# mpetri/ans-large-alphabet

Measured on AMD Instinct MI355X. Metric: encode+decode Mints/s (uint32), bit-exact vs CPU reference per block, higher is better.
Workload: dtype u32 symbols; ANS state carried as an exact f64 (integers below 2^53) in the encoder, u64 in the decoder; 1 GPU; ANSfold-1 on 268435456 uint32 per GPU, zipf20s1.2, blocks of 16384 ints, restart every 1024; codec=ANSfold-1, ints_per_gpu=268435456, distribution=zipf20s1.2, block_ints=16384, ckpt_interval=1024, seed=1234, multi_gpu=single GPU

## Files before the change

### ans_large_alphabet_amd/csrc/ansx.hip

```cpp
#include "../../include/ansx.h"

#include <hip/hip_runtime.h>
#include <dlfcn.h>
#include <rccl/rccl.h>

#include <algorithm>
#include <array>
#include <cmath>
#include <cstdio>
#include <cstdlib>
#include <cstring>
#include <deque>
#include <functional>
#include <map>
#include <set>
#include <string>
#include <vector>

#include "ansx_kernels.h"
#include "ansx_rfold.h"
#include "ansx_model.h"
#include "ansx_fastmodel.h"
#include "ansx_gen.h"
#include "ansx_pa.h"
// ... 67 lines not shown
    std::vector<hipEvent_t> pipe_ev;
    struct {
        bool table16_fixup = false;
        bool encode_gtab16 = false;
        bool parse_generic = false;
        bool parse_win = false;
        bool parse_fast = false;
        bool decode_table = false;
        bool no_stream_lds = false;
        int decode_mode = 0;
        u32 parse_stage_words = 0;
        bool model_fused = false;
        bool model_sync = false;
        bool use_pc = false;
        u32 pc_b_pairs = 2;
        u32 test_sp_bits = 0;
        bool fin_one_wave = false;
        bool no_big_geo = false;
        bool no_pc_auto = false;
        bool encode_mode2 = false;
        bool force_pc = false;
        bool no_pc = false;
        int decode_small_ring = 0;
        int decode_pair = 0;
        u32 pair_lds_limit = 0;
        u32 wide_at = 16;
        bool wide_restart = false;
        u32 ns_hint = 0;
        u32 t_hint = 0;
        bool no_fast_model = false;
        double near_band = ANSX_NEAR_BAND;
        bool near_flip = false;
        u32 cand_chains = 0;
        double fast_guard = ANSX_FAST_GUARD;
        int model_pipeline = 0;
        u32 batch_pass_blocks = 0;
    } dbg;
};

namespace {

#define HIPCHK(ctx, call)                                                                        \
    do {                                                                                         \
        hipError_t _e = (call);                                                                  \
        if (_e != hipSuccess) {                                                                  \
            (ctx)->last_hip = (int)_e;                                                           \
// ... 1171 lines not shown
        const u64 key = geo_key(P.g);
        const size_t stream_bound = block_bound(P.g.kind, P.g.f, P.g.block_ints, P.g.pa != 0) + 16;
        const bool must = P.g.kind == ANSX_INT || stream_bound >= ((size_t)1 << ANSX_CK_CURSOR_BITS) || c->dbg.wide_restart;
        const bool hinted = !must && c->wide_hint.count(key) != 0;
        set_restart_format(&P, must || hinted);
        int rc = encode_dev_once(c, P, d_in, d_out, cap, out_bytes, s);
        if (rc == ANSX_OK && hinted && c->last.max_log2_frame <= c->dbg.wide_at) {
            c->wide_hint.erase(key);
            set_restart_format(&P, false);
            const u32 path0 = c->last.path;
            rc = encode_dev_once(c, P, d_in, d_out, cap, out_bytes, s);
            c->last.path |= (path0 & 16u) | 64u;
        }
        if (rc != ANSX_RETRY_WIDE) return rc;
        c->wide_hint.insert(key);
        set_restart_format(&P, true);
        const int rc2 = encode_dev_once(c, P, d_in, d_out, cap, out_bytes, s);
        c->last.path |= 32u;
        return rc2;
    }
    return encode_dev_once(c, P, d_in, d_out, cap, out_bytes, s);
}

template <bool RF>
int launch_decode(ansx_ctx* c, const ansx_geo& g, u32 NSP, const u8* cont, const u64* boff,
    const u64* ck_state, const u32* ck_off, u64 payload_off, u32* d_out, u32 maxM, u32 max_ns,
    u32 max_block_bytes, u64 cont_bytes, u32* gflags, hipStream_t s, const uint4* pa_info, const u32* hints, u32 max_ep,
    bool parsed = false)
{
    const u32 T = fold_T(g.f);
    int rc;
    if ((rc = ensure(c, c->dec_cum, (size_t)g.nblocks * (NSP + 8) * 4))) return rc;
    if ((rc = ensure(c, c->dec_info, (size_t)g.nblocks * 16))) return rc;
    const size_t pf_e = std::max<size_t>(20480, rup(((size_t)max_ns + 2) * 128, 16));
    const size_t pf_lds = pf_e + (size_t)ANSX_PF_SW * 64 * 4 + 21 * 64 * 4;
    u32 stage_words = ANSX_PF_SW;
    if (c->dbg.parse_stage_words >= 2 && c->dbg.parse_stage_words <= ANSX_PF_SW)
        stage_words = c->dbg.parse_stage_words & ~1u;
    if (parsed) {
    } else if (c->dbg.parse_generic) {
        LAUNCH(c, "k_parse_prelude", (k_parse_prelude<RF>), (g.nblocks + 63) / 64, 64, 0, s, cont, g, NSP,
            boff, payload_off, max_ns, maxM, (u32*)c->dec_cum.p, (uint4*)c->dec_info.p, gflags, pa_info);
    } else if (hints != nullptr && !c->dbg.parse_win && !c->dbg.parse_fast) {
        const u32 par_waves = (g.nblocks + 7) / 8;
        const u32 pw_max = max_ns <= 1024 ? 3u : 4u;
        const u32 pw = std::min<u32>(pw_max, std::max<u32>(1u, (par_waves + c->num_cus - 1) / c->num_cus));
        const u32 par_grid = (par_waves + pw - 1) / pw;
        const size_t lds = (size_t)pw * (32 + 48) * 64 * 4;
        HIPCHK(c, hipFuncSetAttribute((const void*)k_parse_prelude_par<RF, 32>,
                      hipFuncAttributeMaxDynamicSharedMemorySize, (int)lds));
        LAUNCH(c, "k_parse_prelude", (k_parse_prelude_par<RF, 32>), par_grid, 64 * pw, lds, s, cont, g, NSP, boff,
            payload_off, max_ns, maxM, hints, (u32*)c->dec_cum.p, (uint4*)c->dec_info.p, gflags, pa_info);
    } else if (c->dbg.parse_fast && (u64)maxM + max_ns + 3 <= 65535u && pf_lds <= 150 * 1024) {
        HIPCHK(c, hipFuncSetAttribute((const void*)k_parse_prelude_fast<RF>,
                      hipFuncAttributeMaxDynamicSharedMemorySize, (int)pf_lds));
        LAUNCH(c, "k_parse_prelude", (k_parse_prelude_fast<RF>), (g.nblocks + 63) / 64, 64, pf_lds, s, cont, g,
            NSP, boff, payload_off, max_ns, maxM, (u32*)c->dec_cum.p, (uint4*)c->dec_info.p, gflags, stage_words, pa_info);
    } else if (max_ns <= 1024) {
        const size_t lds = (size_t)(128 + 72) * 64 * 4;
        HIPCHK(c, hipFuncSetAttribute((const void*)k_parse_prelude_win<RF, 128>,
                      hipFuncAttributeMaxDynamicSharedMemorySize, (int)lds));
        LAUNCH(c, "k_parse_prelude", (k_parse_prelude_win<RF, 128>), (g.nblocks + 63) / 64, 64, lds, s, cont, g,
            NSP, boff, payload_off, max_ns, maxM, (u32*)c->dec_cum.p, (uint4*)c->dec_info.p, gflags, pa_info);
    } else {
        const size_t lds = (size_t)(256 + 72) * 64 * 4;
        HIPCHK(c, hipFuncSetAttribute((const void*)k_parse_prelude_win<RF, 256>,
                      hipFuncAttributeMaxDynamicSharedMemorySize, (int)lds));
        LAUNCH(c, "k_parse_prelude", (k_parse_prelude_win<RF, 256>), (g.nblocks + 63) / 64, 64, lds, s, cont, g,
            NSP, boff, payload_off, max_ns, maxM, (u32*)c->dec_cum.p, (uint4*)c->dec_info.p, gflags, pa_info);
    }
    const u32 nseg = geo_nseg(g.block_ints, g.ckpt);
    u32 threads = (u32)rup((size_t)nseg * 4, 64);
    if (threads > 256) threads = 256;
    const size_t mfb = RF ? (size_t)T * 4 : 0;
    const size_t want_stream = rup((size_t)max_block_bytes + 32, 16);
    const size_t LDS_LIMIT = 150 * 1024;
    const size_t rs_tables = rup((size_t)(maxM >= 32 ? maxM / 32 : 1) * 8, 16) + 2 * rup((size_t)max_ep * 4, 16) + ANSX_DEC_SCRATCH;
    if (maxM <= 65536u && rs_tables <= LDS_LIMIT && !c->dbg.decode_table) {
        const size_t ring_lds = (size_t)(threads / 4) * ANSX_RING_STRIDE + 16;
        const bool staged_fits = rs_tables + want_stream <= 52 * 1024;
        const bool ring_ok = g.ckpt != 0 && g.block_ints % g.ckpt == 0 && g.ckpt % 4 == 0
            && rs_tables + ring_lds <= 60 * 1024;
        const bool ring_pays = !staged_fits || rs_tables >= 12 * 1024
            || 10 * (rs_tables + want_stream) > 16 * (rs_tables + ring_lds);
        const int force = c->dbg.decode_mode;
        const bool use_ring = ring_ok && (force ? force == 1 : ring_pays);
        if (use_ring) {
            const size_t lds2 = rup((size_t)(maxM >= 32 ? maxM / 32 : 1) * 16, 16) + 4 * rup((size_t)max_ep * 4, 16) + ANSX_DEC_SCRATCH + 2 * ring_lds;
            const int pair = c->dbg.decode_pair;
            if (pair != 1 && g.nblocks >= 2 && (pair == 2 ? lds2 <= 150 * 1024 : lds2 <= c->dbg.pair_lds_limit)) {
                if (lds2 > 48 * 1024)
                    HIPCHK(c, hipFuncSetAttribute((const void*)k_decode_rank2<RF>,
                                  hipFuncAttributeMaxDynamicSharedMemorySize, (int)lds2));
                LAUNCH(c, "k_decode", (k_decode_rank2<RF>), (g.nblocks + 1) / 2, threads, lds2, s, cont, g, NSP, boff,
                    ck_state, ck_off, payload_off, d_out, maxM, max_ep, (u64)cont_bytes, (const u32*)c->dec_cum.p,
                    (const uint4*)c->dec_info.p, gflags);
                return ANSX_OK;
            }
            const int small = c->dbg.decode_small_ring;
            const bool lean = g.n != 0 && (double)(cont_bytes - payload_off) / (double)g.n <= 2.0 && g.ckpt % 16 == 0;
            if (small != 1 && (small == 2 || lean)) {
                const size_t ldss = rs_tables + (size_t)(threads / 4) * ANSX_SRING_STRIDE + 16;
                if (ldss > 48 * 1024)
                    HIPCHK(c, hipFuncSetAttribute((const void*)k_decode_rank<RF, 2>, hipFuncAttributeMaxDynamicSharedMemorySize, (int)ldss));
                LAUNCH(c, "k_decode", (k_decode_rank<RF, 2>), g.nblocks, threads, ldss, s, cont, g, NSP, boff,
                    ck_state, ck_off, payload_off, d_out, maxM, max_ep, (u64)cont_bytes, (const u32*)c->dec_cum.p,
                    (const uint4*)c->dec_info.p, gflags);
                return ANSX_OK;
            }
            const size_t lds = rs_tables + ring_lds;
            if (lds > 48 * 1024)
                HIPCHK(c, hipFuncSetAttribute((const void*)k_decode_rank<RF, 1>,
                              hipFuncAttributeMaxDynamicSharedMemorySize, (int)lds));
            LAUNCH(c, "k_decode", (k_decode_rank<RF, 1>), g.nblocks, threads, lds, s, cont, g, NSP, boff,
                ck_state, ck_off, payload_off, d_out, maxM, max_ep, (u64)cont_bytes, (const u32*)c->dec_cum.p,
                (const uint4*)c->dec_info.p, gflags);
            return ANSX_OK;
        }
        size_t lds = rs_tables;
        u32 stream_cap = 0;
        if (staged_fits && !c->dbg.no_stream_lds) {
            lds += want_stream;
            stream_cap = (u32)want_stream;
        }
        if (lds > 48 * 1024)
            HIPCHK(c, hipFuncSetAttribute((const void*)k_decode_rank<RF, 0>,
                          hipFuncAttributeMaxDynamicSharedMemorySize, (int)lds));
        LAUNCH(c, "k_decode", (k_decode_rank<RF, 0>), g.nblocks, threads, lds, s, cont, g, NSP, boff, ck_state,
            ck_off, payload_off, d_out, maxM, max_ep, (u64)stream_cap, (const u32*)c->dec_cum.p,
            (const uint4*)c->dec_info.p, gflags);
        return ANSX_OK;
    }
    const size_t cb = rup(((size_t)max_ns + 2) * 4, 16);
    const size_t s2sb = rup((size_t)maxM * 2, 16);
    const size_t tables = cb + s2sb + mfb;
    if (tables <= LDS_LIMIT) {
        size_t lds = tables;
        u32 stream_cap = 0;
        if (tables + want_stream <= 52 * 1024) {
            lds += want_stream;
            stream_cap = (u32)want_stream;
        }
        if (lds > 48 * 1024)
            HIPCHK(c, hipFuncSetAttribute((const void*)k_decode<true, RF>,
                          hipFuncAttributeMaxDynamicSharedMemorySize, (int)lds));
        LAUNCH(c, "k_decode_table", (k_decode<true, RF>), g.nblocks, threads, lds, s, cont, g, NSP, boff,
            ck_state, ck_off, payload_off, d_out, maxM, max_ns, stream_cap, (u16*)nullptr,
            (u32*)c->dec_cum.p, (const uint4*)c->dec_info.p, gflags);
    } else {
        if ((rc = ensure(c, c->dec_s2s, (size_t)g.nblocks * maxM * 2))) return rc;
        size_t lds = mfb;
        u32 stream_cap = 0;
        if (mfb + want_stream <= 52 * 1024) {
// ... 1124 lines not shown
    if (hipGetDeviceCount(&ndev) != hipSuccess || ndev == 0) return ANSX_ERR_NO_DEVICE;
    if (device < 0) {
        if (hipGetDevice(&device) != hipSuccess) return ANSX_ERR_NO_DEVICE;
    }
    if (device >= ndev) return ANSX_ERR_ARG;
    if (hipSetDevice(device) != hipSuccess) return ANSX_ERR_NO_DEVICE;
    hipDeviceProp_t prop;
    if (hipGetDeviceProperties(&prop, device) != hipSuccess) return ANSX_ERR_NO_DEVICE;
    if (strncmp(prop.gcnArchName, "gfx950", 6) != 0) return ANSX_ERR_NO_DEVICE;
    ansx_ctx* c = new ansx_ctx();
    c->device = device;
    c->num_cus = prop.multiProcessorCount > 0 ? (u32)prop.multiProcessorCount : 256u;
    if (hipStreamCreateWithFlags(&c->stream, hipStreamDefault) != hipSuccess) {
        delete c;
        return ANSX_ERR_HIP;
    }
    if (hipHostMalloc((void**)&c->h_pin, 4096, hipHostMallocDefault) != hipSuccess) {
        (void)hipStreamDestroy(c->stream);
        delete c;
        return ANSX_ERR_HIP;
    }
    static const char* const names[] = { "ANSX_TEST_TABLE16_FIXUP", "ANSX_ENCODE_GTAB16", "ANSX_PARSE_GENERIC", "ANSX_PARSE_WIN", "ANSX_PARSE_FAST",
        "ANSX_DECODE_TABLE", "ANSX_NO_STREAM_LDS", "ANSX_DECODE_MODE", "ANSX_PARSE_STAGE_WORDS", "ANSX_MODEL_FUSED", "ANSX_MODEL_SYNC", "ANSX_NS_HINT", "ANSX_T_HINT", "ANSX_NO_FAST_MODEL", "ANSX_FAST_GUARD", "ANSX_CAND_CHAINS", "ANSX_NEAR_BAND", "ANSX_TEST_NEAR_FLIP", "ANSX_WIDE_RESTART", "ANSX_TEST_WIDE_AT",
        "ANSX_BATCH_PASS_BLOCKS", "ANSX_MODEL_PIPELINE" };
    for (const char* nm : names)
        if (const char* v = getenv(nm)) (void)ansx_debug_set(c, nm, v);
    *out = c;
    return ANSX_OK;
}

int ansx_last_encode_stats(const ansx_ctx* c, ansx_encode_stats* out)
{
    if (!c || !out) return ANSX_ERR_ARG;
    *out = c->last;
#ifdef ANSX_STAMPS
    {
        static unsigned long long h[16 * 256 + 16];
        if (hipMemcpyFromSymbol(h, HIP_SYMBOL(g_stamps), sizeof(h)) == hipSuccess) {
            double acc[16] = {};
            int nn = 0;
#ifdef ANSX_STAMPS_RF
            const int last = 8;
#else
            const int last = 10;
#endif
            for (int w = 0; w < 256; w++) {
                if (!h[w * 16] || !h[w * 16 + last]) continue;
// ... 40 lines not shown
    else if (!strcmp(name, "ANSX_NO_STREAM_LDS")) c->dbg.no_stream_lds = on;
    else if (!strcmp(name, "ANSX_MODEL_FUSED")) c->dbg.model_fused = on;
    else if (!strcmp(name, "ANSX_MODEL_SYNC")) c->dbg.model_sync = on;
    else if (!strcmp(name, "ANSX_DECODE_MODE"))
        c->dbg.decode_mode = !value ? 0 : !strcmp(value, "ring") ? 1 : !strcmp(value, "staged") ? 2 : 0;
    else if (!strcmp(name, "ANSX_PARSE_STAGE_WORDS")) c->dbg.parse_stage_words = value ? (u32)strtoul(value, nullptr, 10) : 0u;
    else if (!strcmp(name, "ANSX_NS_HINT")) c->dbg.ns_hint = value ? (u32)strtoul(value, nullptr, 10) : 0u;
    else if (!strcmp(name, "ANSX_T_HINT")) c->dbg.t_hint = value ? (u32)strtoul(value, nullptr, 10) : 0u;
    else if (!strcmp(name, "ANSX_NO_FAST_MODEL")) c->dbg.no_fast_model = on;
    else if (!strcmp(name, "ANSX_WIDE_RESTART")) c->dbg.wide_restart = on;
    else if (!strcmp(name, "ANSX_NO_PC")) c->dbg.no_pc = on;
    else if (!strcmp(name, "ANSX_FORCE_PC")) c->dbg.force_pc = on;
    else if (!strcmp(name, "ANSX_USE_PC")) c->dbg.use_pc = on;
    else if (!strcmp(name, "ANSX_NO_PC_AUTO")) c->dbg.no_pc_auto = on;
    else if (!strcmp(name, "ANSX_NO_BIG_GEO")) c->dbg.no_big_geo = on;
    else if (!strcmp(name, "ANSX_FIN_ONE_WAVE")) c->dbg.fin_one_wave = on;
    else if (!strcmp(name, "ANSX_TEST_SP_BITS")) c->dbg.test_sp_bits = value ? (u32)atoi(value) : 0u;
    else if (!strcmp(name, "ANSX_PC_B_PAIRS")) c->dbg.pc_b_pairs = (value && value[0] == '1') ? 1u : 2u;
    else if (!strcmp(name, "ANSX_ENCODE_MODE2")) c->dbg.encode_mode2 = on;
    else if (!strcmp(name, "ANSX_DECODE_SMALL_RING"))
        c->dbg.decode_small_ring = !value ? 0 : !strcmp(value, "never") ? 1 : !strcmp(value, "always") ? 2 : 0;
    else if (!strcmp(name, "ANSX_DECODE_PAIR"))
        c->dbg.decode_pair = !value ? 0 : !strcmp(value, "never") ? 1 : !strcmp(value, "always") ? 2 : 0;
    else if (!strcmp(name, "ANSX_DECODE_PAIR_LDS")) c->dbg.pair_lds_limit = (value && value[0]) ? (u32)strtoul(value, nullptr, 10) : 0u;
    else if (!strcmp(name, "ANSX_FORGET_HINTS")) {
        c->ns_hint.clear();
        c->rf_hint.clear();
        c->t_hint.clear();
        c->wide_hint.clear();
        c->bat.ns_hint.clear(), c->bat.rf_hint.clear(), c->bat.t_hint.clear(), c->bat.wide_hint.clear(), c->bat.int_sparse_hint.clear();
        c->hdr_cache.clear();
        c->hdr_order.clear();
    }
    else if (!strcmp(name, "ANSX_TEST_WIDE_AT")) {
        const u32 v = (value && value[0]) ? (u32)strtoul(value, nullptr, 10) : 16u;
        if (v > 16) return ANSX_ERR_ARG;
        c->dbg.wide_at = v;
    }
    else if (!strcmp(name, "ANSX_NEAR_BAND")) c->dbg.near_band = (value && value[0]) ? strtod(value, nullptr) : ANSX_NEAR_BAND;
    else if (!strcmp(name, "ANSX_TEST_NEAR_FLIP")) c->dbg.near_flip = on;
    else if (!strcmp(name, "ANSX_BATCH_PASS_BLOCKS")) c->dbg.batch_pass_blocks = (value && value[0]) ? (u32)strtoul(value, nullptr, 10) : 0u;
    else if (!strcmp(name, "ANSX_MODEL_PIPELINE")) {
        if (!value || !value[0] || !strcmp(value, "0")) c->dbg.model_pipeline = 0;
        else if (!strcmp(value, "never")) c->dbg.model_pipeline = ANSX_PIPE_NEVER;
        else if (!strcmp(value, "always")) c->dbg.model_pipeline = ANSX_PIPE_ALWAYS;
        else {
// ... 571 lines not shown
```

### ans_large_alphabet_amd/csrc/ansx_kernels.h

```cpp
#pragma once

#include <type_traits>

#include "ansx_dev.h"

#ifdef ANSX_STAMPS
__device__ unsigned long long g_stamps[16 * 256 + 16];
#define STAMP(i) do { if (threadIdx.x == 0 && blockIdx.x % 61 == 7 && blockIdx.x / 61 < 256) g_stamps[(blockIdx.x / 61) * 16 + (i)] = wall_clock64(); } while (0)
#else
#define STAMP(i) do { } while (0)
#endif
#ifdef ANSX_STAMPS_RF
#define STAMP_RF(i) STAMP(i)
#else
#define STAMP_RF(i) do { } while (0)
#endif

struct ansx_blk {
    u32 n;
    u32 max_sym;
    u32 sigma;
    u32 m0_log2;
    double H;
    double thr;
// ... 2559 lines not shown
            sp = sp + (push ? 1u : 0u) - ((pop && sp) ? 1u : 0u);
            const u32 below = sp ? sp - 1 : STK - 1;
            const u32 ra = stkA[below][lane], rl = stkL[below][lane], rh = stkH[below][lane];
            if (pop) {
                ta = ra, tl = rl, th = rh;
            }
            const u32 nbit = go ? bitpos + len : bitpos;
            if ((nbit >> 5) != (bitpos >> 5)) {
                w0 = w1, w1 = w2, w2 = w3;
            }
            bitpos = nbit;
            const u32 rel = (nbit >> 5) - base_w;
            w3 = stage[rel + 3 < SW ? rel + 3 : SW - 1][lane];
            if (__builtin_amdgcn_ballot_w64(go && done < cnt && rel + 5 >= SW) != 0) {
                trigger = true;
                break;
            }
        }
        if (!trigger) break;
    }
    return err;
}

template <bool RFOLD, u32 SW>
__global__ __launch_bounds__(64) void k_parse_prelude_win(const u8* __restrict__ cont, ansx_geo g, u32 NSP,
    const u64* __restrict__ block_off, u64 payload_off, u32 max_ns, u32 maxM,
    u32* __restrict__ g_cum, uint4* __restrict__ binfo, u32* __restrict__ gflags, const uint4* __restrict__ pa_info)
{
    extern __shared__ u32 pw_lds[];
    u32(*stage)[64] = (u32(*)[64])pw_lds;
    u32(*stkA)[64] = (u32(*)[64])(pw_lds + SW * 64);
    u32(*stkL)[64] = stkA + 24;
    u32(*stkH)[64] = stkL + 24;
    const u32 lane = threadIdx.x;
    const u32 b = blockIdx.x * 64 + lane;
    const bool live = b < g.nblocks;
    parse_hdr H;
    H.err = 1, H.ns = 1, H.logM = 0, H.flag = 0, H.pos = 0, H.sbytes = 0, H.stream = cont;
    if (live) H = parse_header<RFOLD>(cont, g, NSP, block_off, payload_off, max_ns, maxM, b, pa_info);
    const u32 herr = H.err;
    const u32 ns = herr ? 0u : H.ns;
    const u8* bp = H.stream + H.pos;
    const u32 avail_words = herr ? 0u : (H.sbytes - H.pos) >> 2;
    const u32 u = (1u << H.logM) + ns + 1;
    u32* cum = g_cum + (u64)(live ? b : 0) * (NSP + 8);
    const u32 err = parse_subtree_win<SW, 24>(stage, stkA, stkL, stkH, lane, bp, avail_words, u, 0, ns, 1, u + 1, 0, herr, cum);
    if (live) {
        binfo[b] = make_uint4(H.ns, H.logM, H.flag, err);
        if (err && herr != 2) atomicOr(&gflags[ANSX_G_ERR], 1u << 3 );
    }
}

template <bool RFOLD, u32 SW>
__global__ __launch_bounds__(256) void k_parse_prelude_par(const u8* __restrict__ cont, ansx_geo g, u32 NSP,
    const u64* __restrict__ block_off, u64 payload_off, u32 max_ns, u32 maxM, const u32* __restrict__ hints,
    u32* __restrict__ g_cum, uint4* __restrict__ binfo, u32* __restrict__ gflags, const uint4* __restrict__ pa_info)
{
    extern __shared__ u32 par_lds[];
    const u32 lane = threadIdx.x & 63, wv = threadIdx.x >> 6;
    u32 (*stage)[64] = (u32 (*)[64])(par_lds + wv * ((SW + 48) * 64));
    u32 (*stkA)[64] = stage + SW;
    u32 (*stkL)[64] = stkA + 16;
    u32 (*stkH)[64] = stkL + 16;
    const u32 j = lane & 7;
    const u32 b = (blockIdx.x * (blockDim.x >> 6) + wv) * 8 + (lane >> 3);
    const bool live = b < g.nblocks;
    parse_hdr H;
    H.err = 1, H.ns = 1, H.logM = 0, H.flag = 0, H.pos = 0, H.sbytes = 0, H.stream = cont;
    if (live) H = parse_header<RFOLD>(cont, g, NSP, block_off, payload_off, max_ns, maxM, b, pa_info);
    const u32 herr = H.err;
    const u32 ns = herr ? 0u : H.ns;
    const u8* bp = H.stream + H.pos;
    const u32 avail_words = herr ? 0u : (H.sbytes - H.pos) >> 2;
    const u32 maxbits = avail_words * 32;
    const u32 u = (1u << H.logM) + ns + 1;
    u32* cum = g_cum + (u64)(live ? b : 0) * (NSP + 8);
// ... 26 lines not shown
            v = low + n1 - 1 + val;
            len = (U == 1) ? 0u : lb + (big ? 1u : 0u);
            if (U == 0 || U > u + 1 || bit + len > maxbits) err = 1;
            else cum[a + h] = v - 1;
        }
        const int src = (int)((lane & ~7u) | (j >> 1));
        const u32 pa_ = (u32)__shfl((int)a, src), pn = (u32)__shfl((int)n, src), plow = (u32)__shfl((int)low, src),
                  phigh = (u32)__shfl((int)high, src), pbit = (u32)__shfl((int)bit, src), pv = (u32)__shfl((int)v, src),
                  plen = (u32)__shfl((int)len, src), perr = (u32)__shfl((int)err, src);
        const u32 hword = (u32)__shfl((int)hv, (int)((lane & ~7u) | (((1u << k) + (j >> 1)) & 7u)));
        if (j < (2u << k)) {
            const u32 ph = (pn + 1) >> 1;
            const bool right = (j & 1u) != 0;
            const bool dead = pn == 0 || perr != 0;
            a = right ? pa_ + ph : pa_;
            n = dead ? 0u : (right ? pn - ph : ph - 1);
            low = right ? pv + 1 : plow;
            high = right ? phigh : pv - 1;
            bit = right ? hword : pbit + plen;
            err = perr;
            if (n != 0 && bit > maxbits) err = 1;
        }
    }
    err = parse_subtree_win<SW, 16>(stage, stkA, stkL, stkH, lane, bp, avail_words, u, a, n, low, high, bit,
        herr ? herr : err, cum);
    u32 e = err;
    e |= (u32)__shfl_xor((int)e, 1);
    e |= (u32)__shfl_xor((int)e, 2);
    e |= (u32)__shfl_xor((int)e, 4);
    if (live && j == 0) {
        binfo[b] = make_uint4(H.ns, H.logM, H.flag, herr == 2 ? 2u : (e ? 1u : 0u));
        if (e && herr != 2) atomicOr(&gflags[ANSX_G_ERR], 1u << 3 );
    }
}

#ifndef ANSX_RING_CHK
#define ANSX_RING_CHK 4
#endif
#define ANSX_DEC_SCRATCH 96u
#define ANSX_RING_BYTES (128 * ANSX_RING_CHK)
#define ANSX_RING_STRIDE (ANSX_RING_BYTES + 16)
#define ANSX_SRING_BYTES 256
#define ANSX_SRING_STRIDE (ANSX_SRING_BYTES + 16)
template <int MODE>
__device__ __forceinline__ u64 dec_fetch8(const u8* __restrict__ stream, const u32* lds_stream, int end8)
{
    if (MODE == 1) {
        const int w = end8 >> 2;
// ... 473 lines not shown
                for (u32 u = 0; u < (u32)CHK; u++) v4[u] = dec_step<3>(st, q, true, qc, logM, mask, Lb, lut, stream, ring);
            }
            quad_transpose4(v4, ql);
            *(ansx_u32x4*)(ob + 4 * (i + ql)) = ansx_u32x4{ v4[0], v4[1], v4[2], v4[3] };
        }
        asm volatile("s_waitcnt vmcnt(0)" : "+v"(rr[0]), "+v"(rr[NP - 1])::"memory");
        if (i < steps) {
            refill_at(ANSX_DEC_P(q));
            for (; i < steps; i++) op[4 * i] = dec_step<3>(st, q, true, qc, logM, mask, Lb, lut, stream, ring);
        }
    }
}

__device__ __forceinline__ void dec_stage_stream(u32* lds_stream, const u8* __restrict__ stream, u32 sbytes,
    u32 tid, u32 nt)
{
    const u32 nw = (sbytes + 3) >> 2;
    for (u32 w = tid; w < nw; w += nt) lds_stream[w + 2] = ld_u32_unaligned(stream + 4 * (u64)w);
    if (tid < 2) lds_stream[tid] = 0;
    if (tid < 2) lds_stream[nw + 2 + tid] = 0;
}

template <bool RFOLD, u32 WSTRIDE, u32 WOFF>
__device__ __forceinline__ bool dec_build_rank_tables(const ansx_geo& g, u32* bw, uint2* ep, u64* sh_scan, u32* sh_bad,
    const u32* __restrict__ gc, u32 (&cur4)[4], u32 (&prv4)[4], u32 ns, u32 M, u32 W, u32 max_ns, u32 rflag,
    const u8* __restrict__ stream, u32 tid, u32 nt, u32* __restrict__ gflags)
{
    const ansx_map f = g.map;
    const u32 T = fold_T(g.f);
    {
        u64 carry = 0;
        u32 bad = 0;
        for (u32 c0 = 0; c0 < ns; c0 += 4 * nt) {
            u32 c4[4], p4[4], nx4[4] = {}, np4[4] = {};
#pragma unroll
            for (u32 q = 0; q < 4; q++) {
                c4[q] = cur4[q];
                p4[q] = (c0 + q * nt + tid) ? prv4[q] + 1u : 0u;
            }
            if (c0 + 4 * nt < ns) {
#pragma unroll
                for (u32 q = 0; q < 4; q++) {
                    const u32 s = c0 + 4 * nt + q * nt + tid;
                    nx4[q] = s < ns ? gc[s + 1] : 0u;
                    np4[q] = s < ns ? gc[s] : 0u;
                }
            }
// ... 39 lines not shown
            atomicOr(&gflags[ANSX_G_ERR], 1u << 3);
        }
    }
    __syncthreads();
    if (*sh_bad) return false;
    if (tid < 64) {
        const u32 per = (W + 63) / 64;
        const u32 lo = tid * per;
        u32 loc = 0;
        for (u32 i = 0; i < per; i++)
            if (lo + i < W) loc += (u32)__builtin_popcount(bw[(lo + i) * WSTRIDE + WOFF]);
        const u32 incl = wave_incl_scan(loc);
        u32 run = incl - loc + ((u32)(size_t)(__attribute__((address_space(3))) const void*)ep / 8u - 1u);
        for (u32 i = 0; i < per; i++)
            if (lo + i < W) {
                bw[(lo + i) * WSTRIDE + WOFF + 1] = run;
                run += (u32)__builtin_popcount(bw[(lo + i) * WSTRIDE + WOFF]);
            }
    }
    __syncthreads();
    return true;
}

template <bool RFOLD, int RING>
__global__ void k_decode_rank(const u8* __restrict__ cont, ansx_geo g, u32 NSP,
    const u64* __restrict__ block_off, const u64* __restrict__ ckpt_state,
    const u32* __restrict__ ckpt_off, u64 payload_off, u32* __restrict__ outp, u32 maxM,
    u32 max_ns, u64 stream_cap, const u32* __restrict__ g_cum, const uint4* __restrict__ binfo,
    u32* __restrict__ gflags)
{
    extern __shared__ __attribute__((aligned(16))) u8 smem[];
    const u32 tid = threadIdx.x, nt = blockDim.x;
    const u32 b = blockIdx.x;
    const u32* gc = g_cum + (u64)b * (NSP + 8);
    u32 cur4[4], prv4[4];
#pragma unroll
    for (u32 q = 0; q < 4; q++) {
        const u32 s = q * nt + tid;
        cur4[q] = s < NSP ? gc[s + 1] : 0u;
        prv4[q] = (s < NSP && s) ? gc[s] : 0u;
    }
    const uint4 bi = binfo[b];
    const u64 boff = block_off[b], boff1 = block_off[b + 1];
    if (bi.w) return;
    const u32 ns = bi.x, logM = bi.y, rflag = bi.z;
    const u32 nb = geo_block_n(g, b);
    const u8* stream = cont + payload_off + boff;
    const u32 sbytes = (u32)(boff1 - boff);
    const u32 M = 1u << logM;
    const u32 wmax = maxM >= 32 ? maxM / 32 : 1;
    u32 off = 0;
    uint2* bwp = (uint2*)(smem + off);
// ... 8 lines not shown
    const bool use_ring = RING && nb == g.block_ints;
    dec_ring_desc D;
    typename std::conditional<RING == 2, dec_sring_pre, dec_ring_pre>::type RP;
    if (use_ring) {
        const u64 sabs = payload_off + boff;
        D.backoff = (int)(sabs < 1024 ? sabs : 1024);
        const u8* base = cont + (sabs - (u64)D.backoff);
        u64 span = (u64)D.backoff + sbytes + 64;
        const u64 room = stream_cap - (sabs - (u64)D.backoff);
        if (span > room) span = room;
        const u64 ba = (u64)(uintptr_t)base;
        D.rsrc = ansx_u32x4{ (u32)ba, (u32)(ba >> 32) & 0xFFFFu, (u32)span, 0x00020000u };
        if constexpr (RING == 2) dec_sring_prefetch(RP, g, b, sbytes, tid, logM, stream, D, ckpt_state, ckpt_off);
        else if constexpr (RING == 1) dec_ring_prefetch(RP, g, b, sbytes, tid, logM, stream, D, ckpt_state, ckpt_off);
    }
    for (u32 w = tid; w < W; w += nt) bwp[w] = make_uint2(0u, 0u);
    if (tid == 0) {
        sh_bad = 0;
        if ((u32)(size_t)(__attribute__((address_space(3))) void*)bwp != 0u) atomicOr(&gflags[ANSX_G_ERR], 1u << 3);
    }
    const bool st_lds = !RING && (sbytes + 24 <= stream_cap);
    if (st_lds) dec_stage_stream(lds_stream, stream, sbytes, tid, nt);
    __syncthreads();
    if (!dec_build_rank_tables<RFOLD, 2, 0>(g, (u32*)bwp, ep, sh_scan, &sh_bad, gc, cur4, prv4, ns, M, W, max_ns, rflag, stream, tid, nt, gflags)) {
        asm volatile("s_waitcnt vmcnt(0)" ::: "memory");
        return;
    }
    dec_lut_rank lut;
    lut.bwp = bwp;
    lut.ep = ep;
    u32* o = outp + geo_block_out(g, b);
    if (use_ring) {
        const u32 labs = (u32)(size_t)(__attribute__((address_space(3))) void*)lds_stream;
        u32* rings = lds_stream + ((((labs + 15u) & ~15u) - labs) >> 2);
        if constexpr (RING == 2) dec_segments_ring_small(g, b, sbytes, tid, nt, logM, lut, stream, rings, D, ckpt_state, ckpt_off, o, RP);
        else if constexpr (RING == 1) dec_segments_ring(g, b, sbytes, tid, nt, logM, lut, stream, rings, D, ckpt_state, ckpt_off, o, RP);
    } else if (st_lds)
        dec_segments<true>(g, b, nb, sbytes, tid, nt, logM, lut, stream, lds_stream, ckpt_state, ckpt_off, o);
    else
        dec_segments<false>(g, b, nb, sbytes, tid, nt, logM, lut, stream, lds_stream, ckpt_state, ckpt_off, o);
}

template <u32 OFF>
struct dec_lut_rank2 {
    static constexpr bool WIDE = false;
    static constexpr u32 OFFSET = OFF;
    __device__ __forceinline__ void get(u32 slot, u32& fr, u32& base, u32& pv) const
// ... 122 lines not shown
        typedef __attribute__((address_space(3))) const u32 lds_cu32;
        const u32 rb = (u32)(size_t)(__attribute__((address_space(3))) const void*)ring;
        lds_cu32* wp = (lds_cu32*)(size_t)(rb + (a & (ANSX_RING_BYTES - 4)));
        t_w0 = wp[0], t_w1 = wp[1], t_w2 = wp[2];
        t_sh = a & 3;
    }
    __device__ __forceinline__ u32 s4()
    {
        const u32 lo = __builtin_amdgcn_alignbyte(t_w1, t_w0, t_sh);
        const u32 hi = __builtin_amdgcn_alignbyte(t_w2, t_w1, t_sh);
        const u32 s_lo = t_rn ? hi : t_nlo, s_hi = t_rn ? t_nlo : t_nhi;
        st = ((u64)s_hi << 32) | s_lo;
        const u32 k = t_pv >> 30;
        const u32 e = (u32)((u64)(t_rn ? lo : hi) >> (32u - 8u * k));
        return (t_pv & ANSX_PV_MASK) + e;
    }
};

template <bool RFOLD>
__global__ __launch_bounds__(256) void k_decode_rank2(const u8* __restrict__ cont, ansx_geo g, u32 NSP,
    const u64* __restrict__ block_off, const u64* __restrict__ ckpt_state,
    const u32* __restrict__ ckpt_off, u64 payload_off, u32* __restrict__ outp, u32 maxM,
    u32 max_ns, u64 cont_bytes, const u32* __restrict__ g_cum, const uint4* __restrict__ binfo,
    u32* __restrict__ gflags)
{
    extern __shared__ __attribute__((aligned(16))) u8 smem[];
    constexpr int RB = ANSX_RING_BYTES, CHK = ANSX_RING_CHK;
    const u32 tid = threadIdx.x, nt = blockDim.x;
    const u32 bA = 2 * blockIdx.x, bB = bA + 1;
    const bool hasB = bB < g.nblocks;
    const u32 bBs = hasB ? bB : bA;
    const u32* gcA = g_cum + (u64)bA * (NSP + 8);
    const u32* gcB = g_cum + (u64)bBs * (NSP + 8);
    u32 curA[4], prvA[4], curB[4], prvB[4];
#pragma unroll
    for (u32 q = 0; q < 4; q++) {
        const u32 s = q * nt + tid;
        curA[q] = s < NSP ? gcA[s + 1] : 0u;
        prvA[q] = (s < NSP && s) ? gcA[s] : 0u;
        curB[q] = s < NSP ? gcB[s + 1] : 0u;
        prvB[q] = (s < NSP && s) ? gcB[s] : 0u;
    }
    const uint4 biA = binfo[bA], biB = binfo[bBs];
    const u64 boffA = block_off[bA], boffA1 = block_off[bA + 1], boffB1 = block_off[bBs + 1];
    const u64 boffB = hasB ? boffA1 : boffA;
    bool okA = biA.w == 0, okB = hasB && biB.w == 0;
    const u32 logMA = biA.y, logMB = biB.y;
    const u32 nbA = geo_block_n(g, bA), nbB = geo_block_n(g, bBs);
    const u8* streamA = cont + payload_off + boffA;
    const u8* streamB = cont + payload_off + boffB;
    const u32 sbA = (u32)(boffA1 - boffA), sbB = (u32)(boffB1 - boffB);
    const u32 MA = 1u << logMA, MB = 1u << logMB;
    const u32 wmax = maxM >= 32 ? maxM / 32 : 1;
    u32 off = 0;
    u32* bw = (u32*)(smem + off);
    off += wmax * 16;
    const u32 epb = 2 * ((max_ns * 4 + 15) & ~15u);
    uint2* epA = (uint2*)(smem + off);
    off += epb;
    uint2* epB = (uint2*)(smem + off);
    off += epb;
    u64* sh_scan = (u64*)(smem + off);
    u32& sh_bad = *(u32*)(smem + off + 80);
    off += ANSX_DEC_SCRATCH;
    u32* lds_rest = (u32*)(smem + off);
    const u32 labs = (u32)(size_t)(__attribute__((address_space(3))) void*)lds_rest;
    u32* ringsA = lds_rest + ((((labs + 15u) & ~15u) - labs) >> 2);
    u32* ringsB = ringsA + (nt >> 2) * (ANSX_RING_STRIDE / 4);
    const u32 WA = MA >= 32 ? MA / 32 : 1, WB = MB >= 32 ? MB / 32 : 1;
    const bool ringA = nbA == g.block_ints, ringB = hasB && nbB == g.block_ints;
    auto make_desc = [&](u64 boff_, u32 sbytes_) {
        dec_ring_desc D;
        const u64 sabs = payload_off + boff_;
        D.backoff = (int)(sabs < 1024 ? sabs : 1024);
        const u8* base = cont + (sabs - (u64)D.backoff);
        u64 span = (u64)D.backoff + sbytes_ + 64;
        const u64 room = cont_bytes - (sabs - (u64)D.backoff);
        if (span > room) span = room;
        const u64 ba = (u64)(uintptr_t)base;
        D.rsrc = ansx_u32x4{ (u32)ba, (u32)(ba >> 32) & 0xFFFFu, (u32)span, 0x00020000u };
        return D;
    };
    dec_ring_desc DA = make_desc(boffA, sbA), DB = make_desc(boffB, sbB);
    dec_ring_pre RPA, RPB;
#pragma unroll
    for (int j = 0; j < RB / 64; j++) RPA.r[j] = RPB.r[j] = ansx_u32x4{ 0u, 0u, 0u, 0u };
    RPA.st = RPB.st = 0;
    RPA.p = RPB.p = RPA.lo = RPB.lo = 0;
    if (okA && ringA) dec_ring_prefetch(RPA, g, bA, sbA, tid, logMA, streamA, DA, ckpt_state, ckpt_off);
    if (okB && ringB) dec_ring_prefetch(RPB, g, bB, sbB, tid, logMB, streamB, DB, ckpt_state, ckpt_off);
    {
        const u32 Wz = (WA > WB ? WA : WB) * 4;
        for (u32 w = tid; w < Wz; w += nt) bw[w] = 0u;
    }
    if (tid == 0) {
        sh_bad = 0;
        if ((u32)(size_t)(__attribute__((address_space(3))) void*)bw != 0u) atomicOr(&gflags[ANSX_G_ERR], 1u << 3);
    }
    __syncthreads();
    if (okA)
        okA = dec_build_rank_tables<RFOLD, 4, 0>(g, bw, epA, sh_scan, &sh_bad, gcA, curA, prvA, biA.x, MA, WA, max_ns, biA.z, streamA, tid, nt, gflags);
    if (okB) {
        if (tid == 0) sh_bad = 0;
        __syncthreads();
        okB = dec_build_rank_tables<RFOLD, 4, 2>(g, bw, epB, sh_scan, &sh_bad, gcB, curB, prvB, biB.x, MB, WB, max_ns, biB.z, streamB, tid, nt, gflags);
    }
    u32* oA = outp + geo_block_out(g, bA);
    u32* oB = outp + geo_block_out(g, bBs);
    dec_lut_rank2<0> lutA;
    dec_lut_rank2<8> lutB;
    if (okA && ringA && okB && ringB) {
        const u32 nseg = g.block_ints / g.ckpt;
        const u32 nq = nt >> 2, quad = tid >> 2, ql = tid & 3;
        const dec_quad_const qc = dec_make_qc(ql);
        const u32 steps = g.ckpt >> 2;
        dec_ring_chain<dec_lut_rank2<0>> A;
        dec_ring_chain<dec_lut_rank2<8>> B;
        A.setup(ringsA, quad, ql, logMA, DA);
        B.setup(ringsB, quad, ql, logMB, DB);
        for (u32 seg = quad; seg < nseg; seg += nq) {
            ansx_u32x4 ra[RB / 64], rb[RB / 64];
            if (seg == quad) {
                A.begin(RPA, ra);
                B.begin(RPB, rb);
            } else {
                A.begin(g, bA, seg, ql, sbA, ckpt_state, ckpt_off, ra);
                B.begin(g, bB, seg, ql, sbB, ckpt_state, ckpt_off, rb);
            }
            asm volatile("s_waitcnt vmcnt(0)" ::: "memory");
// ... 239 lines not shown
```

Before: 144,600 Mints/s.

## Add array-based parse subtree and register-held rank table build for decode setup

Adds a new form of the parallel prelude parser. It keeps decoded endpoints in a per-lane array of u16 or u32 values instead of separate low, high and address stacks, and falls back to the windowed parser when the stage window runs out. It also adds a rank-table build for the decoder that keeps up to 12 entries per thread in registers. That build replaces the chunked scan with a single popcount prefix pass, and it splits the bad flag between the A and B blocks so one barrier is removed. The aim is to cut setup latency in the parse and decode kernels, at the cost of more registers and a wider occupancy setting (pw_max of 4). The old behaviour stays available through the ANSX_DECODE_SETUP=old setting.

```diff
diff --git a/ans_large_alphabet_amd/csrc/ansx.hip b/ans_large_alphabet_amd/csrc/ansx.hip
--- a/ans_large_alphabet_amd/csrc/ansx.hip
+++ b/ans_large_alphabet_amd/csrc/ansx.hip
@@ -113,6 +113,7 @@
         bool force_pc = false;
         bool no_pc = false;
         int decode_small_ring = 0;
+        bool setup_old = false;
         int decode_pair = 0;
         u32 pair_lds_limit = 0;
         u32 wide_at = 16;
@@ -1330,6 +1331,15 @@
     return encode_dev_once(c, P, d_in, d_out, cap, out_bytes, s);
 }
 
+static int ansx_par_form(u32 max_ns, u32 maxM)
+{
+    const size_t room = (size_t)(48 - ANSX_PAR_STK) * 64 * 4;
+    const size_t elems = (size_t)(max_ns >> 3) + 2;
+    if ((u64)maxM + max_ns + 3 <= 65535u && elems * 64 * 2 <= room) return 1;
+    if (elems * 64 * 4 <= room) return 2;
+    return 0;
+}
+
 template <bool RF>
 int launch_decode(ansx_ctx* c, const ansx_geo& g, u32 NSP, const u8* cont, const u64* boff,
     const u64* ck_state, const u32* ck_off, u64 payload_off, u32* d_out, u32 maxM, u32 max_ns,
@@ -1350,15 +1360,23 @@
         LAUNCH(c, "k_parse_prelude", (k_parse_prelude<RF>), (g.nblocks + 63) / 64, 64, 0, s, cont, g, NSP,
             boff, payload_off, max_ns, maxM, (u32*)c->dec_cum.p, (uint4*)c->dec_info.p, gflags, pa_info);
     } else if (hints != nullptr && !c->dbg.parse_win && !c->dbg.parse_fast) {
+        const int form = c->dbg.setup_old ? 0 : ansx_par_form(max_ns, maxM);
         const u32 par_waves = (g.nblocks + 7) / 8;
-        const u32 pw_max = max_ns <= 1024 ? 3u : 4u;
+        const u32 pw_max = (form != 0 || max_ns > 1024) ? 4u : 3u;
         const u32 pw = std::min<u32>(pw_max, std::max<u32>(1u, (par_waves + c->num_cus - 1) / c->num_cus));
         const u32 par_grid = (par_waves + pw - 1) / pw;
-        const size_t lds = (size_t)pw * (32 + 48) * 64 * 4;
-        HIPCHK(c, hipFuncSetAttribute((const void*)k_parse_prelude_par<RF, 32>,
-                      hipFuncAttributeMaxDynamicSharedMemorySize, (int)lds));
-        LAUNCH(c, "k_parse_prelude", (k_parse_prelude_par<RF, 32>), par_grid, 64 * pw, lds, s, cont, g, NSP, boff,
-            payload_off, max_ns, maxM, hints, (u32*)c->dec_cum.p, (uint4*)c->dec_info.p, gflags, pa_info);
+        const size_t lds = (size_t)pw * ANSX_PAR_SLICE_WORDS * 4;
+#define ANSX_LAUNCH_PAR(FORM, label)                                                                                        \
+    do {                                                                                                                    \
+        HIPCHK(c, hipFuncSetAttribute((const void*)k_parse_prelude_par<RF, ANSX_PAR_SW, FORM>,                              \
+                      hipFuncAttributeMaxDynamicSharedMemorySize, (int)lds));                                               \
+        LAUNCH(c, label, (k_parse_prelude_par<RF, ANSX_PAR_SW, FORM>), par_grid, 64 * pw, lds, s, cont, g, NSP, boff,       \
+            payload_off, max_ns, maxM, hints, (u32*)c->dec_cum.p, (uint4*)c->dec_info.p, gflags, pa_info);                  \
+    } while (0)
+        if (form == 1) ANSX_LAUNCH_PAR(1, "k_parse_prelude_arr");
+        else if (form == 2) ANSX_LAUNCH_PAR(2, "k_parse_prelude_arr");
+        else ANSX_LAUNCH_PAR(0, "k_parse_prelude");
+#undef ANSX_LAUNCH_PAR
     } else if (c->dbg.parse_fast && (u64)maxM + max_ns + 3 <= 65535u && pf_lds <= 150 * 1024) {
         HIPCHK(c, hipFuncSetAttribute((const void*)k_parse_prelude_fast<RF>,
                       hipFuncAttributeMaxDynamicSharedMemorySize, (int)pf_lds));
@@ -1383,6 +1401,7 @@
     const size_t mfb = RF ? (size_t)T * 4 : 0;
     const size_t want_stream = rup((size_t)max_block_bytes + 32, 16);
     const size_t LDS_LIMIT = 150 * 1024;
+    const u32 setup_old = c->dbg.setup_old ? 1u : 0u;
     const size_t rs_tables = rup((size_t)(maxM >= 32 ? maxM / 32 : 1) * 8, 16) + 2 * rup((size_t)max_ep * 4, 16) + ANSX_DEC_SCRATCH;
     if (maxM <= 65536u && rs_tables <= LDS_LIMIT && !c->dbg.decode_table) {
         const size_t ring_lds = (size_t)(threads / 4) * ANSX_RING_STRIDE + 16;
@@ -1402,7 +1421,7 @@
                                   hipFuncAttributeMaxDynamicSharedMemorySize, (int)lds2));
                 LAUNCH(c, "k_decode", (k_decode_rank2<RF>), (g.nblocks + 1) / 2, threads, lds2, s, cont, g, NSP, boff,
                     ck_state, ck_off, payload_off, d_out, maxM, max_ep, (u64)cont_bytes, (const u32*)c->dec_cum.p,
-                    (const uint4*)c->dec_info.p, gflags);
+                    (const uint4*)c->dec_info.p, gflags, setup_old);
                 return ANSX_OK;
             }
             const int small = c->dbg.decode_small_ring;
@@ -1413,7 +1432,7 @@
                     HIPCHK(c, hipFuncSetAttribute((const void*)k_decode_rank<RF, 2>, hipFuncAttributeMaxDynamicSharedMemorySize, (int)ldss));
                 LAUNCH(c, "k_decode", (k_decode_rank<RF, 2>), g.nblocks, threads, ldss, s, cont, g, NSP, boff,
                     ck_state, ck_off, payload_off, d_out, maxM, max_ep, (u64)cont_bytes, (const u32*)c->dec_cum.p,
-                    (const uint4*)c->dec_info.p, gflags);
+                    (const uint4*)c->dec_info.p, gflags, setup_old);
                 return ANSX_OK;
             }
             const size_t lds = rs_tables + ring_lds;
@@ -1422,7 +1441,7 @@
                               hipFuncAttributeMaxDynamicSharedMemorySize, (int)lds));
             LAUNCH(c, "k_decode", (k_decode_rank<RF, 1>), g.nblocks, threads, lds, s, cont, g, NSP, boff,
                 ck_state, ck_off, payload_off, d_out, maxM, max_ep, (u64)cont_bytes, (const u32*)c->dec_cum.p,
-                (const uint4*)c->dec_info.p, gflags);
+                (const uint4*)c->dec_info.p, gflags, setup_old);
             return ANSX_OK;
         }
         size_t lds = rs_tables;
@@ -1436,7 +1455,7 @@
                           hipFuncAttributeMaxDynamicSharedMemorySize, (int)lds));
         LAUNCH(c, "k_decode", (k_decode_rank<RF, 0>), g.nblocks, threads, lds, s, cont, g, NSP, boff, ck_state,
             ck_off, payload_off, d_out, maxM, max_ep, (u64)stream_cap, (const u32*)c->dec_cum.p,
-            (const uint4*)c->dec_info.p, gflags);
+            (const uint4*)c->dec_info.p, gflags, setup_old);
         return ANSX_OK;
     }
     const size_t cb = rup(((size_t)max_ns + 2) * 4, 16);
@@ -2607,7 +2626,7 @@
     }
     static const char* const names[] = { "ANSX_TEST_TABLE16_FIXUP", "ANSX_ENCODE_GTAB16", "ANSX_PARSE_GENERIC", "ANSX_PARSE_WIN", "ANSX_PARSE_FAST",
         "ANSX_DECODE_TABLE", "ANSX_NO_STREAM_LDS", "ANSX_DECODE_MODE", "ANSX_PARSE_STAGE_WORDS", "ANSX_MODEL_FUSED", "ANSX_MODEL_SYNC", "ANSX_NS_HINT", "ANSX_T_HINT", "ANSX_NO_FAST_MODEL", "ANSX_FAST_GUARD", "ANSX_CAND_CHAINS", "ANSX_NEAR_BAND", "ANSX_TEST_NEAR_FLIP", "ANSX_WIDE_RESTART", "ANSX_TEST_WIDE_AT",
-        "ANSX_BATCH_PASS_BLOCKS", "ANSX_MODEL_PIPELINE" };
+        "ANSX_BATCH_PASS_BLOCKS", "ANSX_MODEL_PIPELINE", "ANSX_DECODE_SETUP" };
     for (const char* nm : names)
         if (const char* v = getenv(nm)) (void)ansx_debug_set(c, nm, v);
     *out = c;
@@ -2694,6 +2713,11 @@
         c->dbg.decode_small_ring = !value ? 0 : !strcmp(value, "never") ? 1 : !strcmp(value, "always") ? 2 : 0;
     else if (!strcmp(name, "ANSX_DECODE_PAIR"))
         c->dbg.decode_pair = !value ? 0 : !strcmp(value, "never") ? 1 : !strcmp(value, "always") ? 2 : 0;
+    else if (!strcmp(name, "ANSX_DECODE_SETUP")) {
+        if (!value || !value[0] || !strcmp(value, "0")) c->dbg.setup_old = false;
+        else if (!strcmp(value, "old")) c->dbg.setup_old = true;
+        else return ANSX_ERR_ARG;
+    }
     else if (!strcmp(name, "ANSX_DECODE_PAIR_LDS")) c->dbg.pair_lds_limit = (value && value[0]) ? (u32)strtoul(value, nullptr, 10) : 0u;
     else if (!strcmp(name, "ANSX_FORGET_HINTS")) {
         c->ns_hint.clear();
diff --git a/ans_large_alphabet_amd/csrc/ansx_kernels.h b/ans_large_alphabet_amd/csrc/ansx_kernels.h
--- a/ans_large_alphabet_amd/csrc/ansx_kernels.h
+++ b/ans_large_alphabet_amd/csrc/ansx_kernels.h
@@ -2605,6 +2605,81 @@
     return err;
 }
 
+template <u32 SW, u32 STK, typename ET>
+__device__ __forceinline__ u32 parse_subtree_arr(u32 (*stage)[64], u32 (*stack)[64], ET (*E)[64], u32 lane,
+    const u8* __restrict__ bp, u32 avail_words, u32 u, u32 a0, u32 n0, u32 low0, u32 high0, u32 bit0, u32 err,
+    u32* __restrict__ cum, u32& slow)
+{
+    const u32 cnt = err ? 0u : n0;
+    const u32 base_w = bit0 >> 5;
+#pragma unroll 8
+    for (u32 j = 0; j < SW / 2; j++) {
+        const u32 w = base_w + 2 * j;
+        u64 v = 0;
+        if (cnt && w + 2 <= avail_words) v = ld_u64_unaligned(bp + 4 * (u64)w);
+        else if (cnt && w < avail_words) v = ld_u32_unaligned(bp + 4 * (u64)w);
+        stage[2 * j][lane] = (u32)v;
+        stage[2 * j + 1][lane] = (u32)(v >> 32);
+    }
+    const u32 maxbits = cnt ? avail_words * 32 - base_w * 32 : 0u;
+    E[0][lane] = (ET)(low0 - 1);
+    E[cnt + 1][lane] = (ET)(high0 + 1);
+    stack[0][lane] = 0;
+    u32 a = 0, n = cnt, low = low0, high = high0, bitpos = bit0 & 31u, sp = 0, stop = 0;
+    for (u32 it = 0; it < cnt; it++) {
+        const u32 h = (n + 1) >> 1;
+        const u32 n1 = h - 1, n2 = n - h, pe = a + h;
+        const bool caseA = n1 != 0, caseB = !caseA && n2 != 0, caseC = !caseA && !caseB;
+        const u32 pc = stack[sp ? sp - 1 : 0][lane];
+        u32 wi = bitpos >> 5;
+        wi = wi < SW - 2 ? wi : SW - 2;
+        const u32 w0 = stage[wi][lane], w1 = stage[wi + 1][lane];
+        const u32 pa = pc >> 16, pn = pc & 0xFFFFu;
+        const u32 Ea = E[pa][lane], Eb = E[pa + pn + 1][lane];
+        const bool push = caseA && n2 != 0;
+        stack[push ? sp : STK - 1][lane] = (pe << 16) | n2;
+        const u32 U = high - n2 - low - n1 + 1;
+        const u32 win = __builtin_amdgcn_alignbit(w1, w0, bitpos & 31u);
+        const u32 Um1 = U - 1;
+        const u32 bb = 32 - __clz(Um1 | 1u) - (Um1 == 0 ? 1u : 0u);
+        const u32 lb = bb ? bb - 1 : 0;
+        const u32 m = (u32)((1ull << bb) - U);
+        const u32 dh = U - ((1u << lb) & (bb ? ~0u : 0u));
+        u32 val = (win & ((1u << lb) - 1u)) + 1;
+        const bool big = (U != 1) && (val > m);
+        val = big ? (2 * val + ((win >> lb) & 1u)) - m - 1 : val;
+        val += dh;
+        if (val > U) val -= U;
+        if (U == 1) val = 1;
+        const u32 v = low + n1 - 1 + val;
+        const u32 len = (U == 1) ? 0u : lb + (big ? 1u : 0u);
+        const bool bad = (U == 0) || (U > u + 1) || (bitpos + len > maxbits);
+        const u32 now = (bitpos + 64 > SW * 32) ? 2u : (bad ? 1u : 0u);
+        stop = stop ? stop : now;
+        bitpos += stop ? 0u : len;
+        E[pe][lane] = (ET)v;
+        const u32 na = caseA ? a : (caseB ? pe : pa);
+        const u32 nn = caseA ? n1 : (caseB ? n2 : pn);
+        const u32 nlow = caseA ? low : (caseB ? v + 1 : Ea + 1);
+        const u32 nhigh = caseA ? v - 1 : (caseB ? high : Eb - 1);
+        sp = sp + (push ? 1u : 0u) - ((caseC && sp) ? 1u : 0u);
+        a = na, n = nn, low = nlow, high = nhigh;
+    }
+    if (cnt && !stop) {
+        u32* dst = cum + a0 + 1;
+        u32 head = (4u - (u32)(((size_t)dst >> 2) & 3u)) & 3u;
+        head = head < cnt ? head : cnt;
+        u32 i = 0;
+        for (; i < head; i++) dst[i] = (u32)E[i + 1][lane] - 1u;
+        for (; i + 4 <= cnt; i += 4)
+            *(ansx_u32x4*)(dst + i) = ansx_u32x4{ (u32)E[i + 1][lane] - 1u, (u32)E[i + 2][lane] - 1u,
+                (u32)E[i + 3][lane] - 1u, (u32)E[i + 4][lane] - 1u };
+        for (; i < cnt; i++) dst[i] = (u32)E[i + 1][lane] - 1u;
+    }
+    slow = stop == 2 ? 1u : 0u;
+    return stop == 1 ? 1u : err;
+}
+
 template <bool RFOLD, u32 SW>
 __global__ __launch_bounds__(64) void k_parse_prelude_win(const u8* __restrict__ cont, ansx_geo g, u32 NSP,
     const u64* __restrict__ block_off, u64 payload_off, u32 max_ns, u32 maxM,
@@ -2634,7 +2709,10 @@
     }
 }
 
-template <bool RFOLD, u32 SW>
+#define ANSX_PAR_SW 32u
+#define ANSX_PAR_STK 11u
+#define ANSX_PAR_SLICE_WORDS ((ANSX_PAR_SW + 48u) * 64u)
+template <bool RFOLD, u32 SW, int FORM>
 __global__ __launch_bounds__(256) void k_parse_prelude_par(const u8* __restrict__ cont, ansx_geo g, u32 NSP,
     const u64* __restrict__ block_off, u64 payload_off, u32 max_ns, u32 maxM, const u32* __restrict__ hints,
     u32* __restrict__ g_cum, uint4* __restrict__ binfo, u32* __restrict__ gflags, const uint4* __restrict__ pa_info)
@@ -2707,8 +2785,22 @@
             if (n != 0 && bit > maxbits) err = 1;
         }
     }
-    err = parse_subtree_win<SW, 16>(stage, stkA, stkL, stkH, lane, bp, avail_words, u, a, n, low, high, bit,
-        herr ? herr : err, cum);
+    if constexpr (FORM == 0) {
+        err = parse_subtree_win<SW, 16>(stage, stkA, stkL, stkH, lane, bp, avail_words, u, a, n, low, high, bit,
+            herr ? herr : err, cum);
+    } else {
+        typedef typename std::conditional<FORM == 1, u16, u32>::type ET;
+        u32 slow = 0;
+        const u32 e0 = herr ? herr : err;
+        err = parse_subtree_arr<SW, ANSX_PAR_STK, ET>(stage, stkA, (ET (*)[64])(stkA + ANSX_PAR_STK), lane, bp,
+            avail_words, u, a, n, low, high, bit, e0, cum, slow);
+        if (__builtin_amdgcn_ballot_w64(slow != 0) != 0) {
+            wave_lds_sync();
+            const u32 e1 = parse_subtree_win<SW, 16>(stage, stkA, stkL, stkH, lane, bp, avail_words, u, a,
+                slow ? n : 0u, low, high, bit, e0, cum);
+            if (slow) err = e1;
+        }
+    }
     u32 e = err;
     e |= (u32)__shfl_xor((int)e, 1);
     e |= (u32)__shfl_xor((int)e, 2);
@@ -3228,7 +3320,7 @@
 }
 
 template <bool RFOLD, u32 WSTRIDE, u32 WOFF>
-__device__ __forceinline__ bool dec_build_rank_tables(const ansx_geo& g, u32* bw, uint2* ep, u64* sh_scan, u32* sh_bad,
+__device__ __forceinline__ bool dec_build_rank_tables_scan(const ansx_geo& g, u32* bw, uint2* ep, u64* sh_scan, u32* sh_bad,
     const u32* __restrict__ gc, u32 (&cur4)[4], u32 (&prv4)[4], u32 ns, u32 M, u32 W, u32 max_ns, u32 rflag,
     const u8* __restrict__ stream, u32 tid, u32 nt, u32* __restrict__ gflags)
 {
@@ -3314,12 +3406,109 @@
     return true;
 }
 
+template <bool RFOLD, u32 WSTRIDE, u32 WOFF>
+__device__ __forceinline__ bool dec_build_rank_tables(const ansx_geo& g, u32* bw, uint2* ep, u64* sh_scan, u32* sh_bad,
+    const u32* __restrict__ gc, u32 (&cur4)[4], u32 (&prv4)[4], u32 ns, u32 M, u32 W, u32 max_ns, u32 rflag,
+    const u8* __restrict__ stream, u32 tid, u32 nt, u32* __restrict__ gflags, bool scan_form)
+{
+    if (scan_form || ns > 12 * nt)
+        return dec_build_rank_tables_scan<RFOLD, WSTRIDE, WOFF>(g, bw, ep, sh_scan, sh_bad, gc, cur4, prv4, ns, M, W, max_ns, rflag, stream, tid, nt, gflags);
+    const ansx_map f = g.map;
+    const u32 T = fold_T(g.f);
+    u32 bad = ns == 0 ? 1u : 0u;
+    auto entry = [&](u32 c, u32 pg, u32 s) -> u32 {
+        const u32 p = s ? pg + 1u : 0u;
+        const u32 fr = c - p;
+        if (c < p || fr > M || fr > 0xFFFFu) {
+            bad = 1;
+            return 0u;
+        }
+        const u32 base = s ? pg - (s - 1u) : 0u;
+        if (s == ns - 1 && (u64)base + fr != M) bad = 1;
+        if (!fr) return 0u;
+        if (!(base < M && base + fr <= M)) {
+            bad = 1;
+            return 0u;
+        }
+        return (base << 16) | fr;
+    };
+    u32 keep[12];
+#pragma unroll
+    for (u32 q = 0; q < 12; q++) keep[q] = 0u;
+#pragma unroll
+    for (u32 ch = 0; ch < 3; ch++) {
+        const u32 c0 = ch * 4 * nt;
+        if (c0 >= ns) break;
+        u32 nx4[4] = {}, np4[4] = {};
+        if (ch < 2 && c0 + 4 * nt < ns) {
+#pragma unroll
+            for (u32 q = 0; q < 4; q++) {
+                const u32 s = c0 + 4 * nt + q * nt + tid;
+                nx4[q] = s < ns ? gc[s + 1] : 0u;
+                np4[q] = s < ns ? gc[s] : 0u;
+            }
+        }
+#pragma unroll
+        for (u32 q = 0; q < 4; q++) {
+            const u32 s = c0 + q * nt + tid;
+            if (s < ns) {
+                const u32 pk = entry(cur4[q], prv4[q], s);
+                if (pk) atomicOr(&bw[(pk >> 21) * WSTRIDE + WOFF], 1u << ((pk >> 16) & 31u));
+                keep[4 * ch + q] = pk;
+            }
+        }
+#pragma unroll
+        for (u32 q = 0; q < 4; q++) {
+            cur4[q] = nx4[q];
+            prv4[q] = np4[q];
+        }
+    }
+    __syncthreads();
+    if (tid < 64) {
+        const u32 per = (W + 63) / 64;
+        const u32 lo = tid * per;
+        u32 loc = 0;
+        for (u32 i = 0; i < per; i++)
+            if (lo + i < W) loc += (u32)__builtin_popcount(bw[(lo + i) * WSTRIDE + WOFF]);
+        const u32 incl = wave_incl_scan(loc);
+        u32 run = incl - loc + ((u32)(size_t)(__attribute__((address_space(3))) const void*)ep / 8u - 1u);
+        for (u32 i = 0; i < per; i++)
+            if (lo + i < W) {
+                bw[(lo + i) * WSTRIDE + WOFF + 1] = run;
+                run += (u32)__builtin_popcount(bw[(lo + i) * WSTRIDE + WOFF]);
+            }
+    }
+    __syncthreads();
+    const u32 ep8 = (u32)(size_t)(__attribute__((address_space(3))) const void*)ep / 8u;
+#pragma unroll
+    for (u32 q = 0; q < 12; q++) {
+        const u32 pk = keep[q], s = q * nt + tid;
+        if (!pk) continue;
+        const u32 base = pk >> 16;
+        const u32 wd = bw[(base >> 5) * WSTRIDE + WOFF], pf = bw[(base >> 5) * WSTRIDE + WOFF + 1];
+        const u32 r = (u32)__builtin_popcount(wd << (~base & 31u)) + pf - ep8;
+        if (r < max_ns) {
+            u32 mfv = 0;
+            if (RFOLD && rflag && s < T) mfv = ld_u32_unaligned(stream + 4 + 4 * (u64)s);
+            ep[r] = make_uint2(pk, dec_make_pv(f, s, RFOLD && rflag, T, mfv));
+        } else {
+            bad = 1;
+        }
+    }
+    if (bad) {
+        *sh_bad = 1;
+        atomicOr(&gflags[ANSX_G_ERR], 1u << 3);
+    }
+    __syncthreads();
+    return *sh_bad == 0;
+}
+
 template <bool RFOLD, int RING>
 __global__ void k_decode_rank(const u8* __restrict__ cont, ansx_geo g, u32 NSP,
     const u64* __restrict__ block_off, const u64* __restrict__ ckpt_state,
     const u32* __restrict__ ckpt_off, u64 payload_off, u32* __restrict__ outp, u32 maxM,
     u32 max_ns, u64 stream_cap, const u32* __restrict__ g_cum, const uint4* __restrict__ binfo,
-    u32* __restrict__ gflags)
+    u32* __restrict__ gflags, u32 setup_old)
 {
     extern __shared__ __attribute__((aligned(16))) u8 smem[];
     const u32 tid = threadIdx.x, nt = blockDim.x;
@@ -3374,7 +3563,7 @@
     const bool st_lds = !RING && (sbytes + 24 <= stream_cap);
     if (st_lds) dec_stage_stream(lds_stream, stream, sbytes, tid, nt);
     __syncthreads();
-    if (!dec_build_rank_tables<RFOLD, 2, 0>(g, (u32*)bwp, ep, sh_scan, &sh_bad, gc, cur4, prv4, ns, M, W, max_ns, rflag, stream, tid, nt, gflags)) {
+    if (!dec_build_rank_tables<RFOLD, 2, 0>(g, (u32*)bwp, ep, sh_scan, &sh_bad, gc, cur4, prv4, ns, M, W, max_ns, rflag, stream, tid, nt, gflags, setup_old != 0)) {
         asm volatile("s_waitcnt vmcnt(0)" ::: "memory");
         return;
     }
@@ -3543,7 +3732,7 @@
     const u64* __restrict__ block_off, const u64* __restrict__ ckpt_state,
     const u32* __restrict__ ckpt_off, u64 payload_off, u32* __restrict__ outp, u32 maxM,
     u32 max_ns, u64 cont_bytes, const u32* __restrict__ g_cum, const uint4* __restrict__ binfo,
-    u32* __restrict__ gflags)
+    u32* __restrict__ gflags, u32 setup_old)
 {
     extern __shared__ __attribute__((aligned(16))) u8 smem[];
     constexpr int RB = ANSX_RING_BYTES, CHK = ANSX_RING_CHK;
@@ -3583,6 +3772,7 @@
     off += epb;
     u64* sh_scan = (u64*)(smem + off);
     u32& sh_bad = *(u32*)(smem + off + 80);
+    u32& sh_badB = *(u32*)(smem + off + 84);
     off += ANSX_DEC_SCRATCH;
     u32* lds_rest = (u32*)(smem + off);
     const u32 labs = (u32)(size_t)(__attribute__((address_space(3))) void*)lds_rest;
@@ -3616,16 +3806,14 @@
     }
     if (tid == 0) {
         sh_bad = 0;
+        sh_badB = 0;
         if ((u32)(size_t)(__attribute__((address_space(3))) void*)bw != 0u) atomicOr(&gflags[ANSX_G_ERR], 1u << 3);
     }
     __syncthreads();
     if (okA)
-        okA = dec_build_rank_tables<RFOLD, 4, 0>(g, bw, epA, sh_scan, &sh_bad, gcA, curA, prvA, biA.x, MA, WA, max_ns, biA.z, streamA, tid, nt, gflags);
-    if (okB) {
-        if (tid == 0) sh_bad = 0;
-        __syncthreads();
-        okB = dec_build_rank_tables<RFOLD, 4, 2>(g, bw, epB, sh_scan, &sh_bad, gcB, curB, prvB, biB.x, MB, WB, max_ns, biB.z, streamB, tid, nt, gflags);
-    }
+        okA = dec_build_rank_tables<RFOLD, 4, 0>(g, bw, epA, sh_scan, &sh_bad, gcA, curA, prvA, biA.x, MA, WA, max_ns, biA.z, streamA, tid, nt, gflags, setup_old != 0);
+    if (okB)
+        okB = dec_build_rank_tables<RFOLD, 4, 2>(g, bw, epB, sh_scan, &sh_badB, gcB, curB, prvB, biB.x, MB, WB, max_ns, biB.z, streamB, tid, nt, gflags, setup_old != 0);
     u32* oA = outp + geo_block_out(g, bA);
     u32* oB = outp + geo_block_out(g, bBs);
     dec_lut_rank2<0> lutA;
```

Result: faster. 149,900 Mints/s (median of 6 runs) (+3.7%).
